# kianmcevoy/audio_analysis

Measured on AMD Instinct MI355X. Metric: IRs/sec full report (STFT+RT60bands+zplane), 48 kHz 10 s IR, higher is better.
Workload: dtype f64; 1 GPU; metrics-only full report on 256 mono synthetic IRs per GPU per step, 10 s @ 48 kHz (SURVEY.md 8d generator), H2D included: every step uploads its batch from pinned host memory (float32, 492 MB) on a copy stream under the previous step's kernels; 4 distinct batches rotate; batch_per_gpu=256, parallelism=file-sharded dp1, gather=final

## Files before the change

### audio_analysis_amd/csrc/ira_fftlong.hip

```cpp
#include <cmath>
#include <cstdlib>
#include <type_traits>

#include "ira_bandmask.h"
#include "ira_fft_lds.h"

namespace {

using ira::cplx;
typedef cplx<double> cd;

constexpr int FL_THREADS = 256;
constexpr int FL_LR = 4;

struct Geom {
  long long m;
  int n1, rad, log2q, log2n2;
  const cd* t1;
  const cd* t2;
  const cd* tf;
  int ablate;
};

__device__ __forceinline__ unsigned col_slot(const Geom& g, unsigned r) {
// ... 173 lines not shown
constexpr int FL_U = 8;

template <int MODE>
__device__ __forceinline__ RawL fetch_input(const Jobs& J, const Ctx& c, unsigned n) {
  RawL r{0.0, 0.0, 0.0, 0.0, 0.0f, 0.0f};
  if (MODE == IN_SIGNAL) {
    r.fa = c.p1[n < c.lim1 ? c.stu * n : 0u];
    r.fb = c.p2[n < c.lim2 ? c.stu * n : 0u];
  } else if (MODE == IN_SPECTRUM) {
    const unsigned k = n > c.Lu / 2 ? c.Lu - n : n;
    const unsigned kk = n < c.Lu ? k : 0u;
    const cd xk = c.s1[kk];
    r.a = xk.re; r.b = xk.im;
    if (c.two) {
      const cd x2 = c.s2[kk];
      r.c = x2.re; r.d = x2.im;
    }
  }
  return r;
}

template <int MODE>
__device__ __forceinline__ cd value_input(const Jobs& J, const Ctx& c, unsigned n, unsigned M, cd w, double h,
                                          double h2, const RawL& r, bool hann, bool second) {
  const unsigned L = c.Lu;
  if (MODE == IN_SIGNAL) {
    double v = (double)(n < c.lim1 ? r.fa : 0.0f), v2 = (double)(n < c.lim2 ? r.fb : 0.0f);
    if (hann) {
      v *= h; v2 *= h2;
    }
    if (!second) return {v * w.re, v * w.im};
    return {v * w.re - v2 * w.im, v * w.im + v2 * w.re};
  } else if (MODE == IN_FILTER) {
    unsigned m = M - n;
    if (m >= L) {
      m = n;
      if (m >= L) return {0.0, 0.0};
    }
    const cd wm = chirp((long long)m, chirp_scale((long long)L));
    return {wm.re, -wm.im};
  } else {
    if (n >= L) return {0.0, 0.0};
    const bool upper = n > L / 2;
    const unsigned k = upper ? L - n : n;
    const bool self = k == 0u || 2u * k == L;
    const cd xk = {r.a, self ? 0.0 : (upper ? -r.b : r.b)};
    const double m1 = (double)ira::mask_cut(c.b1, c.k1, (int)k, c.fv);
    const double m2 = (double)ira::mask_cut(c.b2, c.k2, (int)k, c.fv);
    cd wk;
    if (!c.two) {
      wk = ira::cmul(xk, cd{m1, m2});
    } else {
      const cd x2 = {r.c, self ? 0.0 : (upper ? -r.d : r.d)};
      wk = {xk.re * m1 - x2.im * m2, xk.im * m1 + x2.re * m2};
    }
    const cd cw = {wk.re, -wk.im};
    return ira::cmul(cw, w);
  }
}

template <int MODE>
__global__ __launch_bounds__(FL_THREADS) __attribute__((amdgpu_waves_per_eu(4, 4))) void cols_fwd_kernel(Geom g, Jobs J, cd* __restrict__ work, int C) {
  extern __shared__ __attribute__((aligned(16))) unsigned char smem_raw[];
  cd* lds = reinterpret_cast<cd*>(smem_raw);
  unsigned bx, by;
  ira::xcd_remap(bx, by);
  const int e = (int)by + J.e0;
  const Ctx ctx = job_ctx<MODE>(J, e);
  const long long L = ctx.L;
  const unsigned N1 = (unsigned)g.n1, N2 = 1u << g.log2n2;
  const long long M = g.m;
  const unsigned n2_0 = bx * C;
  const unsigned lc = 31u - (unsigned)__builtin_clz((unsigned)C), cm = (unsigned)C - 1u;
  const unsigned stride = (unsigned)g.rad * ((1u << g.log2q) + 1u);
  const int tid = threadIdx.x;
  cd* twl = lds + (size_t)C * stride;
  const cd twv = ira::tw_split_fetch<double>(g.t1, N1 >> 1, tid);
  {
    const unsigned c = tid & cm, n1_0 = tid >> lc;
    const unsigned dn = (FL_THREADS >> lc) * N2;
    const unsigned n0 = n1_0 * N2 + n2_0 + c;
    const unsigned total = N1 * (unsigned)C;
    const unsigned cnt_mine = total > (unsigned)tid ? (total - (unsigned)tid + FL_THREADS - 1) / FL_THREADS : 0u;
    auto load_phase = [&](auto known, const unsigned cnt) __attribute__((always_inline)) {
      constexpr int KNOWN = decltype(known)::value;
      constexpr int UI = (MODE == IN_SIGNAL) ? 2 * FL_UI : FL_UI;
      RawL raw[UI];
      if (cnt > 0) {
  #pragma unroll
        for (int u = 0; u < UI; ++u) {
          const unsigned j = (unsigned)u < cnt ? (unsigned)u : cnt - 1;
          raw[u] = fetch_input<MODE>(J, ctx, n0 + j * dn);
        }
      }
      cd w = {1.0, 0.0}, d = {1.0, 0.0}, e2 = {1.0, 0.0};
      long long lw1 = L, lw2 = L;
      if (MODE == IN_SIGNAL) {
        lw1 = ctx.lw1;
        lw2 = ctx.lw2;
      }
      const bool second = (KNOWN & 4) ? (MODE == IN_SIGNAL && ctx.o2 >= 0) : (KNOWN & 2) != 0;
      const bool hann = (KNOWN & 4) ? (MODE == IN_SIGNAL && J.use_hann) : (KNOWN & 1) != 0;
      const bool win1 = (KNOWN & 4) ? lw1 > 1 : true, win2 = (KNOWN & 4) ? lw2 > 1 : true;
      double hc = 1.0, hs = 0.0, rc = 1.0, rs = 0.0, hc2 = 1.0, hs2 = 0.0, rc2 = 1.0, rs2 = 0.0;
      if (MODE != IN_FILTER) {
        const ChirpScale cs = chirp_scale(L);
        const double n0d = (double)n0, dnd = (double)dn;
        w = unit_q(n0d * n0d, cs);
        d = unit_q(2.0 * n0d * dnd + dnd * dnd, cs);
        const double st = (double)ctx.st;
        const double inv1 = win1 ? 1.0 / (double)(lw1 - 1) : 0.0, inv2 = win2 ? 1.0 / (double)(lw2 - 1) : 0.0;
        {
          const int lane = tid & 63;
          const double a = lane == 0 ? chirp_angle(2.0 * dnd * dnd, cs) : (2.0 * st * dnd) * (lane == 1 ? inv1 : inv2);
          double s3, c3;
          sincospi(a, &s3, &c3);
          e2 = {lane_value(c3, 0), -lane_value(s3, 0)};
          if (hann && win1) { rs = lane_value(s3, 1); rc = lane_value(c3, 1); }
          if (hann && second && win2) { rs2 = lane_value(s3, 2); rc2 = lane_value(c3, 2); }
        }
        if (hann) {
          const double i1 = st * n0d, i2 = st * n0d + (st - 1.0);
          if (win1) sincospi((2.0 * i1 + 1.0 - (double)lw1) * inv1, &hs, &hc);
          if (second && win2) sincospi((2.0 * i2 + 1.0 - (double)lw2) * inv2, &hs2, &hc2);
        }
      }
      if (MODE == IN_SIGNAL) {
  #pragma unroll
        for (int u = 0; u < UI; ++u) asm volatile("" : "+v"(raw[u].fa), "+v"(raw[u].fb));
      }
      __builtin_amdgcn_sched_barrier(0);
      for (unsigned jb = 0; jb < cnt; jb += UI) {
        if (jb > 0) {
  #pragma unroll
          for (int u = 0; u < UI; ++u) {
            const unsigned j = jb + u < cnt ? jb + u : cnt - 1;
            raw[u] = fetch_input<MODE>(J, ctx, n0 + j * dn);
          }
        }
  #pragma unroll
        for (int u = 0; u < UI; ++u) {
          const unsigned j = jb + u;
          if (j < cnt) {
            const unsigned n1 = (tid + FL_THREADS * j) >> lc;
            const unsigned n = n0 + j * dn;
            const double h = win1 ? 0.5 + 0.5 * hc : 1.0;
            const double h2 = win2 ? 0.5 + 0.5 * hc2 : 1.0;
            lds[c * stride + col_slot(g, n1)] = (IRA_ABL(g.ablate & 1)) ? cd{(double)n, 1.0} : value_input<MODE>(J, ctx, n, (unsigned)M, w, h, h2, raw[u], hann, second);
            w = ira::cmul(w, d);
            d = ira::cmul(d, e2);
            if (hann) {
              const double nc = hc * rc - hs * rs;
              hs = hs * rc + hc * rs;
              hc = nc;
            }
            if (hann && second) {
              const double nc2 = hc2 * rc2 - hs2 * rs2;
              hs2 = hs2 * rc2 + hc2 * rs2;
              hc2 = nc2;
            }
          }
        }
      }
    };
    using std::integral_constant;
    const unsigned cnt_all = total / FL_THREADS;
    if (total % FL_THREADS != 0) {
      load_phase(integral_constant<int, 4>{}, cnt_mine);
    } else if (MODE != IN_SIGNAL) {
      load_phase(integral_constant<int, 4>{}, cnt_all);
    } else {
      const bool two = ctx.o2 >= 0;
      if (!J.use_hann) {
        if (two) load_phase(integral_constant<int, 2>{}, cnt_all); else load_phase(integral_constant<int, 0>{}, cnt_all);
      } else if (ctx.lw1 > 1 && (!two || ctx.lw2 > 1)) {
        if (two) load_phase(integral_constant<int, 3>{}, cnt_all); else load_phase(integral_constant<int, 1>{}, cnt_all);
      } else {
        load_phase(integral_constant<int, 4>{}, cnt_all);
      }
    }
  }
  ira::tw_split_put(twl, twv, tid);
  __syncthreads();
  if (!(IRA_ABL(g.ablate & 2))) {
    if (g.rad == 3) radix3_stage<false>(g, lds, twl, C, stride, tid);
    ira::lds_fft_dif<double, FL_LR, true>(lds, g.log2q, twl, (unsigned)g.rad, tid, FL_THREADS, C * g.rad, (1u << g.log2q) + 1u);
  }
  cd* w = work + (long long)e * M;
  const unsigned total_o = N1 * (unsigned)C;
  for (unsigned base = 0; base < total_o; base += FL_THREADS * FL_UI) {
    cd th[FL_UI], tl[FL_UI];
#pragma unroll
    for (int u = 0; u < FL_UI; ++u) {
      unsigned i = base + tid + FL_THREADS * u;
      i = i < total_o ? i : total_o - 1;
      const unsigned p = (n2_0 + (i & cm)) * row_k1(g, i >> lc);
      th[u] = g.t1[p >> g.log2n2];
      tl[u] = g.tf[p & (N2 - 1u)];
    }
#pragma unroll
    for (int u = 0; u < FL_UI; ++u) {
      const unsigned i = base + tid + FL_THREADS * u;
      if (i >= total_o) continue;
      const unsigned c = i & cm, r = i >> lc;
      const cd v = ira::cmul(lds[c * stride + col_slot(g, r)], ira::cmul(th[u], tl[u]));
      if ((IRA_ABL(g.ablate & 4)) && v.re != 12345.678) continue;
      w[(long long)r * N2 + n2_0 + c] = v;
    }
  }
}

template <int MODE>
__global__ __launch_bounds__(FL_THREADS) __attribute__((amdgpu_waves_per_eu(4, 4))) void rows_kernel(Geom g, Jobs J, cd* __restrict__ work, int R) {
  extern __shared__ __attribute__((aligned(16))) unsigned char smem_raw[];
  cd* lds = reinterpret_cast<cd*>(smem_raw);
  unsigned bx, by;
  ira::xcd_remap(bx, by);
  const int e = (int)by + J.e0;
  const unsigned N2 = 1u << g.log2n2;
  const long long M = g.m;
// ... 45 lines not shown
        unsigned i = base + tid + FL_THREADS * u;
        i = i < total ? i : total - 1;
        const unsigned p = (i & (N2 - 1)) * row_k1(g, r0 + (i >> g.log2n2));
        th[u] = g.t1[p >> g.log2n2];
        tl[u] = g.tf[p & (N2 - 1u)];
      }
#pragma unroll
      for (int u = 0; u < FL_UI; ++u) {
        const unsigned i = base + tid + FL_THREADS * u;
        if (i >= total) continue;
        cd t = ira::cmul(th[u], tl[u]);
        t.im = -t.im;
        const cd v = ira::cmul(lds[i], t);
        if ((IRA_ABL(g.ablate & 128)) && v.re != 12345.678) continue;
        w[i] = v;
      }
    }
  } else {
    for (unsigned i = tid; i < total; i += FL_THREADS) w[i] = lds[i];
  }
}

template <int MODE>
__global__ __launch_bounds__(FL_THREADS) __attribute__((amdgpu_waves_per_eu(4, 4))) void cols_inv_kernel(Geom g, Jobs J, const cd* __restrict__ work, int C) {
  extern __shared__ __attribute__((aligned(16))) unsigned char smem_raw[];
  cd* lds = reinterpret_cast<cd*>(smem_raw);
  unsigned bx, by;
  ira::xcd_remap(bx, by);
  const int e = (int)by + J.e0;
  long long L, out1, out2 = -1;
  bool paired = false;
  {
    const int l = J.L[e];
    if (MODE == OUT_SPECTRUM) {
      const long long x2 = J.x2off ? (long long)J.x2off[e] : -1ll, zo = J.x2off ? (long long)J.zpair_off[e] : 0ll;
      const long long so = J.spec_out_off[e];
      paired = ira::uniform(x2) >= 0;
      out1 = paired ? ira::uniform(zo) : ira::uniform(so);
    } else {
      const long long y1 = J.y1_off[e], y2 = J.y2_off[e];
      out1 = ira::uniform(y1);
      out2 = ira::uniform(y2);
    }
    L = ira::uniform(l);
  }
  const unsigned N1 = (unsigned)g.n1, N2 = 1u << g.log2n2;
  const long long M = g.m;
  const unsigned n2_0 = bx * C;
  const unsigned lc = 31u - (unsigned)__builtin_clz((unsigned)C), cm = (unsigned)C - 1u;
  const unsigned stride = (unsigned)g.rad * ((1u << g.log2q) + 1u);
  const int tid = threadIdx.x;
  const long long n_need = (MODE == OUT_SPECTRUM && !paired) ? L / 2 + 1 : L;
  const cd* w = work + (long long)e * M;
  const unsigned total = N1 * (unsigned)C;
  cd* twl = lds + (size_t)C * stride;
  const cd twv = ira::tw_split_fetch<double>(g.t1, N1 >> 1, tid);
  for (unsigned base = 0; base < total; base += FL_THREADS * FL_U) {
    cd raw[FL_U];
#pragma unroll
    for (int u = 0; u < FL_U; ++u) {
      unsigned i = base + tid + FL_THREADS * u;
      i = i < total ? i : total - 1;
      raw[u] = (IRA_ABL(g.ablate & 256)) ? cd{(double)i, 1.0} : w[(long long)(i >> lc) * N2 + n2_0 + (i & cm)];
    }
#pragma unroll
    for (int u = 0; u < FL_U; ++u) {
      const unsigned i = base + tid + FL_THREADS * u;
      if (i < total) lds[(i & cm) * stride + col_slot(g, i >> lc)] = raw[u];
    }
  }
  ira::tw_split_put(twl, twv, tid);
  __syncthreads();
  if (!(IRA_ABL(g.ablate & 32))) {
    ira::lds_fft_dit<double, FL_LR, true>(lds, g.log2q, twl, (unsigned)g.rad, true, tid, FL_THREADS, C * g.rad, (1u << g.log2q) + 1u);
    if (g.rad == 3) radix3_stage<true>(g, lds, twl, C, stride, tid);
  }
  const double inv_m = 1.0 / (double)M;
  const long long dn = (long long)(FL_THREADS >> lc) * N2;
  const long long n0 = (long long)((unsigned)tid >> lc) * N2 + n2_0 + ((unsigned)tid & cm);
  const ChirpScale cs = chirp_scale(L);
  const double n0d = (double)n0, dnd = (double)dn;
  cd cw = unit_q(n0d * n0d, cs), cdl = unit_q(2.0 * n0d * dnd + dnd * dnd, cs);
  const cd ce2 = unit_q(2.0 * dnd * dnd, cs);
  for (unsigned i = tid; i < N1 * (unsigned)C; i += FL_THREADS) {
    const unsigned c = i & cm, n1 = i >> lc;
    const long long n = (long long)n1 * N2 + n2_0 + c;
    const cd wn = cw;
    cw = ira::cmul(cw, cdl);
    cdl = ira::cmul(cdl, ce2);
    if (n >= n_need) continue;
    cd v = lds[c * stride + col_slot(g, n1)];
    if (!(IRA_ABL(g.ablate & 64))) v = ira::cmul(v, wn);
    if (MODE == OUT_SPECTRUM) {
      v.re *= inv_m; v.im *= inv_m;
      if (paired) {
        J.zpair[out1 + n] = v;
      } else {
        if (n == 0 || (2 * n == L)) v.im = 0.0;
        J.spec_out[out1 + n] = v;
      }
    } else {
      const double sc = inv_m / (double)L;
      J.y[out1 + n] = (float)(v.re * sc);
      if (out2 >= 0) J.y[out2 + n] = (float)(-v.im * sc);
    }
  }
}

__global__ __launch_bounds__(256) void pair_split_kernel(Jobs J) {
  const int e = blockIdx.y;
  if (J.x2off[e] < 0 || (J.interleave && J.interleave[e])) return;
  const long long L = J.L[e];
  const long long k = (long long)blockIdx.x * blockDim.x + threadIdx.x;
  if (k > L / 2) return;
  const cd* z = J.zpair + J.zpair_off[e];
  const long long o1 = J.spec_out_off[e], o2 = J.spec_out_off2[e];
  ira::pair_split_bin(z, L, k, J.spec_out + o1 + k, J.spec_out + o2 + k);
}

__global__ __launch_bounds__(256) void half_split_kernel(Jobs J) {
  const int e = blockIdx.y;
  if (!J.interleave[e]) return;
  const long long L = J.L[e];
  const long long k = (long long)blockIdx.x * blockDim.x + threadIdx.x;
  if (k > L) return;
  const cd* z = J.zpair + J.zpair_off[e];
  J.spec_out[J.spec_out_off[e] + k] = ira::half_split_bin(z, L, k);
}

struct Split { int rad, log2q, log2n2; };

bool split_of(long long m, Split* out) {
  if (m < 16 || m > (1ll << 22)) return false;
  int rad = 1;
  if (m % 3 == 0) { rad = 3; m /= 3; }
  if ((m & (m - 1)) != 0) return false;
  int log2p = 0;
  while ((1ll << log2p) < m) ++log2p;
  int lq;
  if (rad == 1) {
    const int forced = ira_tune_int("IRA_FFT_SPLIT", 0);
    lq = (log2p + 1) / 2;
    if (forced > 0) lq = forced;
    if (lq < 2) lq = 2;
    if (lq > log2p - 2) lq = log2p - 2;
    if (log2p - lq > 13) lq = log2p - 13;
  } else {
    if (log2p < 5) return false;
    lq = (log2p - 1) / 2;
    { const int forced = ira_tune_int("IRA_FFT_SPLIT3", 0); if (forced >= 2 && forced <= log2p - 2) lq = forced; }
    if (log2p - lq > 13) lq = log2p - 13;
  }
  out->rad = rad; out->log2q = lq; out->log2n2 = log2p - lq;
  return true;
}

struct Plan {
  Geom g;
  int C, R;
  size_t lds_cols, lds_rows;
  int C3; size_t lds_cols3;
};

int32_t make_plan(int32_t m, const void* t1, const void* t2, const void* tf, Plan* p) {
  Split sp;
  if (!split_of(m, &sp)) return IRA_E_SIZE;
  p->g.m = m;
// ... 139 lines not shown
```

### audio_analysis_amd/csrc/ira_spectrum.hip

```cpp
#include <cmath>

#include "ira_fft_reg.h"
#include "ira_log.h"
#include "ira_reduce.h"

namespace {

typedef ira::cplx<double> cd;
constexpr double kPi = 3.14159265358979323846;

constexpr int ATAN_TAB = 64;

__device__ __attribute__((noinline)) double atan2_lib(double y, double x) { return atan2(y, x); }
__device__ __attribute__((noinline)) double fmod_lib(double a, double b) { return fmod(a, b); }
__device__ __attribute__((noinline)) double exp10_lib(double y) { return exp10(y); }
__device__ __attribute__((noinline)) cd twiddle_lib(long long k, long long l) {
  double sn, cs;
  sincospi(-(double)(k % (2 * l)) / (double)l, &sn, &cs);
  return {cs, sn};
}
__device__ __attribute__((noinline)) float db_lib(double re, double im, double floor_lin) {
  const double a = hypot(re, im);
  const double m = (a != a) ? a : fmax(a, floor_lin);
  return (float)(20.0 * log10(m));
}

__device__ __forceinline__ void build_atan_table(double* tab, int tid) {
  if (tid <= ATAN_TAB) tab[tid] = atan((double)tid * (1.0 / ATAN_TAB));
}

__device__ __forceinline__ double atan2_table(double y, double x, const double* tab) {
  const double ax = fabs(x), ay = fabs(y);
  const double mx = fmax(ax, ay), mn = fmin(ax, ay);
  if (!(ax > 1.0e-300 && ay > 1.0e-300 && ax < 1.0e300 && ay < 1.0e300)) return atan2_lib(y, x);
  const double t = mn / mx;
  const int k = (int)(t * (double)ATAN_TAB + 0.5);
  const double t0 = (double)k * (1.0 / ATAN_TAB);
  const double r = (t - t0) / fma(t, t0, 1.0);
  const double r2 = r * r;
  double s = fma(r2, 1.0 / 9.0, -1.0 / 7.0);
  s = fma(r2, s, 0.2);
  s = fma(r2, s, -1.0 / 3.0);
  s = fma(r2, s, 1.0);
  double a = fma(r, s, tab[k]);
  if (ay > ax) a = 1.5707963267948966 - a;
  if (x < 0.0) a = kPi - a;
  return copysign(a, y);
}

__device__ __forceinline__ double unwrap_correction(double prev, double cur) {
  const double dd = cur - prev;
  const double period = 2.0 * kPi;
  double a = dd + kPi;
  double md;
  if (a >= 0.0 && a < period) md = a;
  else if (a >= period && a < 2.0 * period) md = a - period;
  else if (a < 0.0 && a > -period) md = a;
  else md = fmod_lib(a, period);
  if (md != 0.0) {
    if (md < 0.0) md += period;
  } else {
    md = 0.0;
  }
  double ddmod = md + (-kPi);
  if (ddmod == -kPi && dd > 0.0) ddmod = kPi;
  double corr = ddmod - dd;
  if (fabs(dd) < kPi) corr = 0.0;
  return corr;
}

__device__ __forceinline__ cd packed_bin(cd zk, cd zl, double cs, double sn, bool edge) {
  const auto [ev, od] = ira::hermitian_parts(zk, zl);
  cd v = {ev.re + (cs * od.re - sn * od.im), ev.im + (cs * od.im + sn * od.re)};
  if (edge) v.im = 0.0;
  return v;
}

__device__ __forceinline__ float bin_db(cd v, double floor_lin, double floor_p, float floor_db32,
                                        const ira::LogTabEntry* ltab) {
  const double p = v.re * v.re + v.im * v.im;
  if (p > 1.0e-280 && p < 1.0e280 && floor_lin > 1.0e-140) {
    return p > floor_p ? (float)(3.0102999566398120 * ira::log2_table(p, ltab)) : floor_db32;
  }
  return db_lib(v.re, v.im, floor_lin);
}

__global__ __launch_bounds__(256) void mag_phase_kernel(const cd* __restrict__ spec, const int64_t* __restrict__ spec_off,
                                 const int32_t* __restrict__ L, double floor_lin, float* __restrict__ mag_db,
                                 const int64_t* __restrict__ mag_off, double* __restrict__ phase,
                                 const int64_t* __restrict__ phase_off, const int32_t* __restrict__ packed) {
  __shared__ ira::LogTabEntry ltab[ira::LOGTAB_N];
  __shared__ double atab[ATAN_TAB + 1];
  ira::build_log_table(ltab, threadIdx.x);
  build_atan_table(atab, threadIdx.x);
  __syncthreads();
  const int e = blockIdx.y;
  const long long nb = (long long)L[e] / 2 + 1;
  const cd* s = spec + spec_off[e];
  float* mo = mag_db + mag_off[e];
  double* po = phase ? phase + phase_off[e] : nullptr;
  const double floor_p = floor_lin * floor_lin;
  const float floor_db32 = (float)(20.0 * log10(floor_lin));
  const bool pk = packed != nullptr && ira::uniform(packed[e]) != 0;
  const long long l = (long long)L[e] / 2;
  const long long k_first = (long long)blockIdx.x * blockDim.x + threadIdx.x, k_step = (long long)gridDim.x * blockDim.x;
  double cs = 1.0, sn = 0.0, rc = 1.0, rs = 0.0;
  if (pk) {
    sincospi(-(double)(k_first < nb ? k_first : 0) / (double)l, &sn, &cs);
    sincospi(-(double)(k_step % (2 * l)) / (double)l, &rs, &rc);
  }
  for (long long k = k_first; k < nb; k += k_step) {
    cd v;
    if (pk) {
      v = packed_bin(s[k == l ? 0 : k], s[(k == 0 || k == l) ? 0 : l - k], cs, sn, k == 0 || k == l);
      const double nc = cs * rc - sn * rs;
      sn = sn * rc + cs * rs;
      cs = nc;
    } else {
      v = s[k];
    }
    mo[k] = bin_db(v, floor_lin, floor_p, floor_db32, ltab);
// ... 226 lines not shown
      __syncthreads();
    }
    if (compacted) {
#pragma unroll
      for (int r = 0; r < OS_MAX_RANKS; ++r) {
        if (!lead[r]) continue;
        const int li = list_of[r];
        const int cnt = list_n[li] < OS_CAP ? list_n[li] : OS_CAP;
        for (int i = tid; i < cnt; i += OS_THREADS) {
          const unsigned long long k = os_key(list[li][i]);
          if ((k & himask) == pf[r]) atomicAdd(&hist[r][(unsigned int)(k >> shift) & 255u], 1u);
        }
      }
    } else {
      for (long long it = 0; it < trips; ++it) {
        unsigned long long kk[OS_U];
        bool vv[OS_U];
#pragma unroll
        for (int u = 0; u < OS_U; ++u) {
          const long long i = (it * OS_U + u) * OS_THREADS + tid;
          vv[u] = i < n;
          kk[u] = os_key(v[vv[u] ? i : n - 1]);
        }
#pragma unroll
        for (int u = 0; u < OS_U; ++u) {
          const bool valid = vv[u];
          const unsigned long long k = kk[u];
          const unsigned int digit = (unsigned int)(k >> shift) & 255u;
#pragma unroll
          for (int r = 0; r < OS_MAX_RANKS; ++r) {
            if (!lead[r]) continue;
            const bool m = valid && (k & himask) == pf[r];
            const unsigned long long act = __ballot(m);
            if (act == 0ull) continue;
            const int first = __ffsll((long long)act) - 1;
            const unsigned int d0 = (unsigned int)__shfl((int)digit, first, 64);
            const unsigned long long same = __ballot(m && digit == d0);
            if (lane == first) atomicAdd(&hist[r][d0], (unsigned int)__popcll(same));
            if (m && digit != d0) atomicAdd(&hist[r][digit], 1u);
          }
        }
      }
    }
    __syncthreads();
    for (int r = 0; r < nranks; ++r) {
      const int l = leader[r];
      const long long rem = remaining[r];
      const long long c = tid < 256 ? (long long)hist[l][tid] : 0ll;
      long long in_wave;
      long long incl = ira::wave_prefix(c, lane, in_wave);
      if (tid < 256 && lane == 63) scan_tot[tid >> 6] = incl;
      __syncthreads();
      if (tid < 256) {
        for (int w = 0; w < (tid >> 6); ++w) incl += scan_tot[w];
        const long long excl = incl - c;
        if ((excl <= rem && rem < incl) || (tid == 255 && rem >= incl)) {
          remaining[r] = rem - excl;
          bucket[r] = c;
          prefix[r] = prefix[r] | ((unsigned long long)tid << shift);
        }
      }
      __syncthreads();
    }
  }
  if (tid < nranks) o[tid] = os_unkey(prefix[tid]);
}

constexpr int ST_THREADS = 1024;

struct StatsAcc {
  double cnt = 0.0, sfl = 0.0, sl = 0.0;
  unsigned long long best = 0ull;
  unsigned long long near = ~0ull;
  long long first_in;
  float near_db = 0.0f;
};
struct StatsScratch {
  double red[3][ST_THREADS / IRA_WAVE];
  unsigned long long kred[2][ST_THREADS / IRA_WAVE];
  long long lred[ST_THREADS / IRA_WAVE];
  float dred[ST_THREADS / IRA_WAVE];
};

__device__ __forceinline__ void stats_bin(StatsAcc& a, long long k, float db, double val, float f_min, float f_max,
                                          float probe_hz, const double* etab) {
  const float f = (float)((double)k * val);
  const float d = fabsf(f - probe_hz);
  const unsigned long long nk = ((unsigned long long)__float_as_uint(d) << 32) | (unsigned long long)(uint32_t)k;
  a.near_db = nk < a.near ? db : a.near_db;
  a.near = nk < a.near ? nk : a.near;
  if (f >= f_min && f <= f_max) {
    uint32_t uu = ira::float_key(db);
    if (db != db) uu = 0xFFFFFFFFu;
    const unsigned long long key = ((unsigned long long)uu << 32) | (unsigned long long)(0xFFFFFFFFu - (uint32_t)k);
    a.best = key > a.best ? key : a.best;
    const double y = (double)db * 0.05;
    const double lin = fabs(y) < 15.0 ? ira::exp10_table(y, etab) : exp10_lib(y);
    a.cnt += 1.0; a.sfl += (double)f * lin; a.sl += lin;
    a.first_in = k < a.first_in ? k : a.first_in;
  }
}

__device__ __forceinline__ void stats_finish(StatsAcc a, StatsScratch& sc, long long n, double val, double* o) {
  const int t = threadIdx.x, lane = t & 63, wave = t >> 6;
  a.cnt = ira::wave_sum(a.cnt); a.sfl = ira::wave_sum(a.sfl); a.sl = ira::wave_sum(a.sl);
#pragma unroll
  for (int o2 = 32; o2 > 0; o2 >>= 1) {
    const unsigned long long ob = __shfl_xor(a.best, o2, 64);
    a.best = ob > a.best ? ob : a.best;
    const unsigned long long on = __shfl_xor(a.near, o2, 64);
    const float od = __shfl_xor(a.near_db, o2, 64);
    a.near_db = on < a.near ? od : a.near_db;
    a.near = on < a.near ? on : a.near;
    const long long of = __shfl_xor(a.first_in, o2, 64);
    a.first_in = of < a.first_in ? of : a.first_in;
  }
  if (lane == 0) {
    sc.red[0][wave] = a.cnt; sc.red[1][wave] = a.sfl; sc.red[2][wave] = a.sl;
    sc.kred[0][wave] = a.best; sc.kred[1][wave] = a.near; sc.lred[wave] = a.first_in; sc.dred[wave] = a.near_db;
  }
  __syncthreads();
  if (t == 0) {
    a.cnt = a.sfl = a.sl = 0.0;
    for (int w = 0; w < ST_THREADS / IRA_WAVE; ++w) {
      a.cnt += sc.red[0][w]; a.sfl += sc.red[1][w]; a.sl += sc.red[2][w];
      a.best = sc.kred[0][w] > a.best ? sc.kred[0][w] : a.best;
      a.near_db = sc.kred[1][w] < a.near ? sc.dred[w] : a.near_db;
      a.near = sc.kred[1][w] < a.near ? sc.kred[1][w] : a.near;
      a.first_in = sc.lred[w] < a.first_in ? sc.lred[w] : a.first_in;
    }
    const long long pk = (a.cnt > 0.0) ? (long long)(0xFFFFFFFFu - (uint32_t)(a.best & 0xFFFFFFFFull)) : 0;
    o[0] = a.cnt;
    o[1] = (double)pk;
    o[2] = (double)(float)((double)pk * val);
    o[3] = a.sfl; o[4] = a.sl;
    o[5] = a.first_in < n ? (double)(float)((double)a.first_in * val) : 0.0;
    o[6] = (double)(long long)(a.near & 0xFFFFFFFFull);
    o[7] = (double)a.near_db;
  }
}

__global__ __launch_bounds__(ST_THREADS) void stats_kernel(const float* __restrict__ mag_db,
                                                           const int64_t* __restrict__ mag_off,
                                                           const int32_t* __restrict__ L,
                                                           const double* __restrict__ freq_val, float f_min, float f_max,
                                                           float probe_hz, double* __restrict__ out) {
  __shared__ StatsScratch sc;
  __shared__ double etab[ira::EXPTAB_N];
  const int e = blockIdx.x;
  const long long n = (long long)L[e] / 2 + 1;
  const float* m = mag_db + mag_off[e];
  const double val = freq_val[e];
  const int t = threadIdx.x;
  ira::build_exp_table(etab, t);
  __syncthreads();
  StatsAcc acc;
  acc.first_in = n;
  constexpr int ST_U = 16;
  for (long long k0 = t; k0 < n; k0 += (long long)ST_THREADS * ST_U) {
    float dbv[ST_U];
#pragma unroll
    for (int u = 0; u < ST_U; ++u) {
      const long long k = k0 + (long long)ST_THREADS * u;
      dbv[u] = m[k < n ? k : n - 1];
    }
#pragma unroll
    for (int u = 0; u < ST_U; ++u) {
      const long long k = k0 + (long long)ST_THREADS * u;
      if (k >= n) continue;
      stats_bin(acc, k, dbv[u], val, f_min, f_max, probe_hz, etab);
    }
  }
  stats_finish(acc, sc, n, val, out + (int64_t)e * 8);
}

constexpr int SF_TWQ = 512;
constexpr int SF_STAGE = 2;

template <bool DB, bool PHASE>
__global__ __launch_bounds__(UW_THREADS) void spectrum_finish_kernel(
    const cd* __restrict__ spec, const int64_t* __restrict__ spec_off, const int32_t* __restrict__ L, double floor_lin,
    const int32_t* __restrict__ packed, float* __restrict__ mag_db, const int64_t* __restrict__ out_off, int do_unwrap,
    double out_scale, float* __restrict__ phase32, double* __restrict__ phase64, double* __restrict__ wrapped64,
    const double* __restrict__ freq_val, float f_min, float f_max, float probe_hz, double* __restrict__ stats) {
  static_assert(ST_THREADS == UW_THREADS, "the statistics' thread mapping is the tile's load mapping");
  __shared__ ira::LogTabEntry ltab[ira::LOGTAB_N];
  __shared__ double atab[ATAN_TAB + 1];
  __shared__ double etab[ira::EXPTAB_N];
  __shared__ StatsScratch sc;
  __shared__ cd twq[SF_TWQ];
  __shared__ double ph_tile[UW_TILE];
  __shared__ double wave_tot[UW_THREADS / IRA_WAVE];
  __shared__ double tile_total, prev_last;
  const int e = blockIdx.x;
  const int t = threadIdx.x, lane = t & 63, wave = t >> 6;
  const long long len = ira::uniform(L[e]);
  const long long n = len / 2 + 1, l = len / 2;
  const cd* s = spec + ira::uniform(spec_off[e]);
  const long long oo = ira::uniform(out_off[e]);
  const bool pk = packed != nullptr && ira::uniform(packed[e]) != 0 && l > 0;
  const bool want_stats = DB && stats != nullptr;
  const double val = want_stats ? ira::uniform(freq_val[e]) : 0.0;
  const double floor_p = floor_lin * floor_lin;
  const float floor_db32 = (float)(20.0 * log10(floor_lin));
  if constexpr (DB) ira::build_log_table(ltab, t);
  if constexpr (PHASE) build_atan_table(atab, t);
  if (want_stats) ira::build_exp_table(etab, t);
  double wt_c = 1.0, wt_s = 0.0;
  auto build_twq = [&](long long q0) {
    const long long k = (q0 + t) * UW_THREADS;
    if (t < SF_TWQ && k < n) twq[t] = twiddle_lib(k, l);
  };
  if (pk) {
    const cd wt = twiddle_lib(t, l);
    wt_c = wt.re;
    wt_s = wt.im;
    build_twq(0);
  }
  if (t == 0) { tile_total = 0.0; prev_last = 0.0; }
  __syncthreads();
  StatsAcc acc;
  acc.first_in = n;
  cd nza[SF_STAGE], nzb[SF_STAGE];
  auto load_stage = [&](long long first) {
#pragma unroll
    for (int r = 0; r < SF_STAGE; ++r) {
      const long long k = first + t + (long long)UW_THREADS * r;
      nza[r] = {0.0, 0.0};
      nzb[r] = {0.0, 0.0};
      if (k < n) {
        if (pk) {
          nza[r] = s[k == l ? 0 : k];
          nzb[r] = s[(k == 0 || k == l) ? 0 : l - k];
        } else {
          nza[r] = s[k];
        }
      }
    }
  };
  load_stage(0);
  for (long long base = 0; base < n; base += UW_TILE) {
    if (pk && base > 0 && base % ((long long)SF_TWQ * UW_THREADS) == 0) {
      __syncthreads();
      build_twq(base / UW_THREADS);
      __syncthreads();
    }
    const long long qb = base / ((long long)SF_TWQ * UW_THREADS) * SF_TWQ;
#pragma unroll 1
    for (int h = 0; h < UW_PER / SF_STAGE; ++h) {
      const long long first = base + (long long)h * SF_STAGE * UW_THREADS;
      cd za[SF_STAGE], zb[SF_STAGE];
#pragma unroll
      for (int r = 0; r < SF_STAGE; ++r) { za[r] = nza[r]; zb[r] = nzb[r]; }
      if (first + SF_STAGE * UW_THREADS < n) load_stage(first + SF_STAGE * UW_THREADS);
#pragma unroll
      for (int r = 0; r < SF_STAGE; ++r) {
        const int j = t + UW_THREADS * (h * SF_STAGE + r);
        const long long k = base + j;
        double ph = 0.0;
        if (k < n) {
          cd v = za[r];
          if (pk) {
            const cd w = twq[k / UW_THREADS - qb];
            const double cs = w.re * wt_c - w.im * wt_s;
            const double sn = w.im * wt_c + w.re * wt_s;
            v = packed_bin(za[r], zb[r], cs, sn, k == 0 || k == l);
          }
          if constexpr (DB) {
            const float db = bin_db(v, floor_lin, floor_p, floor_db32, ltab);
            mag_db[oo + k] = db;
            if (want_stats) stats_bin(acc, k, db, val, f_min, f_max, probe_hz, etab);
          }
          if constexpr (PHASE) {
            ph = atan2_table(v.im, v.re, atab);
            if (wrapped64) wrapped64[oo + k] = ph;
          }
        }
        if constexpr (PHASE) ph_tile[j] = ph;
      }
    }
    if constexpr (PHASE) {
      __syncthreads();
      const double carry = tile_total;
      const long long i0 = base + (long long)UW_PER * t;
      double c[UW_PER], v[UW_PER];
      double prev = t == 0 ? prev_last : ph_tile[UW_PER * t - 1];
#pragma unroll
      for (int r = 0; r < UW_PER; ++r) v[r] = ph_tile[UW_PER * t + r];
#pragma unroll
      for (int r = 0; r < UW_PER; ++r) {
        const long long i = i0 + r;
        c[r] = (do_unwrap && i >= 1 && i < n) ? unwrap_correction(prev, v[r]) : 0.0;
        prev = v[r];
      }
      const double add = unwrap_scan(c, carry, wave_tot, lane, wave);
#pragma unroll
      for (int r = 0; r < UW_PER; ++r) {
        const long long i = i0 + r;
        if (i < n) {
          const double u = v[r] + (c[r] + add);
          if (phase32) phase32[oo + i] = (float)(u * out_scale);
          if (phase64) phase64[oo + i] = u;
        }
      }
      if (t == UW_THREADS - 1) { tile_total = c[3] + add; prev_last = v[3]; }
    }
  }
  if (want_stats) stats_finish(acc, sc, n, val, stats + (int64_t)e * 8);
}

constexpr int LS_MAX = 2048;
constexpr int LS_THREADS = 256;

__device__ __forceinline__ double ls_freq(long long k, double fstep) { return (double)(float)((double)k * fstep); }

__global__ __launch_bounds__(LS_THREADS) void log_smooth_kernel(float* __restrict__ mag, const int64_t* __restrict__ off,
                                                                const int32_t* __restrict__ stride_a,
                                                                const int32_t* __restrict__ k_lo_a,
                                                                const int32_t* __restrict__ nsel_a,
                                                                const double* __restrict__ fstep_a,
                                                                const double* __restrict__ lg_lo, const double* __restrict__ lg_hi,
                                                                const int32_t* __restrict__ count_a, int window,
                                                                int through_f32) {
  __shared__ double xg[LS_MAX], on[LS_MAX], sm[LS_MAX];
  const int c = blockIdx.x, tid = threadIdx.x;
  const int count = count_a[c], nsel = nsel_a[c], k_lo = k_lo_a[c];
  const long long stride = stride_a[c];
  const double fstep = fstep_a[c], a = lg_lo[c], b = lg_hi[c];
  if (count < 2 || count > LS_MAX || nsel < 1) return;
  float* m = mag + off[c];
  const double step = (b - a) / (double)(count - 1);
  for (int g = tid; g < count; g += LS_THREADS) {
    const double y = (g == count - 1) ? b : (double)g * step + a;
    const double x = exp2(y);
    xg[g] = x;
    double v;
    const double f0 = ls_freq(k_lo, fstep), fl = ls_freq((long long)k_lo + nsel - 1, fstep);
    if (nsel == 1 || x <= f0) v = (double)m[(long long)k_lo * stride];
    else if (x >= fl) v = (double)m[(long long)(k_lo + nsel - 1) * stride];
    else {
      int lo = 0, hi = nsel - 1;
      while (hi - lo > 1) {
        const int mid = (lo + hi) >> 1;
        if (ls_freq((long long)k_lo + mid, fstep) <= x) lo = mid; else hi = mid;
      }
      const double x0 = ls_freq((long long)k_lo + lo, fstep), x1 = ls_freq((long long)k_lo + lo + 1, fstep);
      const double y0 = (double)m[(long long)(k_lo + lo) * stride], y1 = (double)m[(long long)(k_lo + lo + 1) * stride];
      const double slope = (y1 - y0) / (x1 - x0);
      v = slope * (x - x0) + y0;
    }
    on[g] = through_f32 ? (double)(float)v : v;
  }
  __syncthreads();
  const double inv_w = 1.0 / (double)window;
  const int h = (window - 1) / 2;
  for (int g = tid; g < count; g += LS_THREADS) {
    int j0 = g + h - (window - 1), j1 = g + h;
    if (j0 < 0) j0 = 0;
    if (j1 > count - 1) j1 = count - 1;
    double acc = 0.0;
    for (int j = j0; j <= j1; ++j) acc += on[j] * inv_w;
    sm[g] = through_f32 ? (double)(float)acc : acc;
  }
  __syncthreads();
  for (int i = tid; i < nsel; i += LS_THREADS) {
    const double x = ls_freq((long long)k_lo + i, fstep);
    double v;
    if (x <= xg[0]) v = sm[0];
    else if (x >= xg[count - 1]) v = sm[count - 1];
    else {
      int lo = 0, hi = count - 1;
      while (hi - lo > 1) {
        const int mid = (lo + hi) >> 1;
        if (xg[mid] <= x) lo = mid; else hi = mid;
      }
      const double slope = (sm[lo + 1] - sm[lo]) / (xg[lo + 1] - xg[lo]);
      v = slope * (x - xg[lo]) + sm[lo];
    }
    m[(long long)(k_lo + i) * stride] = (float)v;
  }
}

}

extern "C" int32_t ira_spectrum_mag_phase(const double* spec_dev, const int64_t* spec_off_dev, const int32_t* L_dev,
// ... 110 lines not shown
```

Before: 17730 IRs/s.

## Skip zero-padding loads and unneeded output rows; cheapen atan2 and index math

In the long FFT input stage, threads now stop fetching the signal past the data region and write zeros directly to LDS for padded rows. In the output stage, loop trip counts are clamped to the rows actually needed. Separately, the table-based atan2 uses a hardware reciprocal and a division-reduced formulation, and the spectrum kernel switches its index math from 64-bit to 32-bit with precomputed output base pointers. The approximate reciprocal may slightly change phase rounding, and the int indices assume bin counts fit in 32 bits.

```diff
diff --git a/audio_analysis_amd/csrc/ira_fftlong.hip b/audio_analysis_amd/csrc/ira_fftlong.hip
--- a/audio_analysis_amd/csrc/ira_fftlong.hip
+++ b/audio_analysis_amd/csrc/ira_fftlong.hip
@@ -279,16 +279,35 @@
     const unsigned n0 = n1_0 * N2 + n2_0 + c;
     const unsigned total = N1 * (unsigned)C;
     const unsigned cnt_mine = total > (unsigned)tid ? (total - (unsigned)tid + FL_THREADS - 1) / FL_THREADS : 0u;
-    auto load_phase = [&](auto known, const unsigned cnt) __attribute__((always_inline)) {
+    unsigned pad_j = ~0u;
+    static_assert(FL_THREADS == 256, "the shift by 8 - lc below divides by FL_THREADS / C");
+    if (MODE == IN_SIGNAL && !(IRA_ABL(g.ablate & 1))) {
+      const unsigned data = ctx.lim1 > ctx.lim2 ? ctx.lim1 : ctx.lim2;
+      const unsigned rows_data = data > n2_0 ? (data - n2_0 + N2 - 1u) >> g.log2n2 : 0u;
+      const unsigned row_min = ira::uniform(n1_0);
+      pad_j = rows_data > row_min ? (rows_data - row_min + (FL_THREADS >> lc) - 1u) >> (8u - lc) : 0u;
+    }
+    auto load_phase = [&](auto known, const unsigned cnt_own) __attribute__((always_inline)) {
       constexpr int KNOWN = decltype(known)::value;
+      const unsigned cnt = cnt_own < pad_j ? cnt_own : pad_j;
       constexpr int UI = (MODE == IN_SIGNAL) ? 2 * FL_UI : FL_UI;
       RawL raw[UI];
-      if (cnt > 0) {
+      const unsigned cnt_w = MODE == IN_SIGNAL ? ira::uniform(cnt) : 0u;
+      if (MODE == IN_SIGNAL) {
+  #pragma unroll
+        for (int u = 0; u < UI; ++u) {
+          raw[u] = RawL{0.0, 0.0, 0.0, 0.0, 0.0f, 0.0f};
+          if ((unsigned)u < cnt_w) raw[u] = fetch_input<MODE>(J, ctx, n0 + ((unsigned)u < cnt ? (unsigned)u : (cnt ? cnt - 1 : 0u)) * dn);
+        }
+      } else if (cnt > 0) {
   #pragma unroll
         for (int u = 0; u < UI; ++u) {
           const unsigned j = (unsigned)u < cnt ? (unsigned)u : cnt - 1;
           raw[u] = fetch_input<MODE>(J, ctx, n0 + j * dn);
         }
+      }
+      if (MODE == IN_SIGNAL) {
+        for (unsigned j = cnt; j < cnt_own; ++j) lds[c * stride + col_slot(g, (tid + FL_THREADS * j) >> lc)] = cd{0.0, 0.0};
       }
       cd w = {1.0, 0.0}, d = {1.0, 0.0}, e2 = {1.0, 0.0};
       long long lw1 = L, lw2 = L;
@@ -332,7 +351,7 @@
   #pragma unroll
           for (int u = 0; u < UI; ++u) {
             const unsigned j = jb + u < cnt ? jb + u : cnt - 1;
-            raw[u] = fetch_input<MODE>(J, ctx, n0 + j * dn);
+            if (MODE != IN_SIGNAL || jb + u < cnt_w) raw[u] = fetch_input<MODE>(J, ctx, n0 + j * dn);
           }
         }
   #pragma unroll
@@ -544,7 +563,15 @@
   const double n0d = (double)n0, dnd = (double)dn;
   cd cw = unit_q(n0d * n0d, cs), cdl = unit_q(2.0 * n0d * dnd + dnd * dnd, cs);
   const cd ce2 = unit_q(2.0 * dnd * dnd, cs);
-  for (unsigned i = tid; i < N1 * (unsigned)C; i += FL_THREADS) {
+  const unsigned need_u = (unsigned)n_need;
+  const unsigned rows_need = need_u > n2_0 ? (need_u - n2_0 + N2 - 1u) >> g.log2n2 : 0u;
+  const unsigned row_min = ira::uniform((unsigned)tid >> lc);
+  static_assert(FL_THREADS == 256, "the shift by 8 - lc divides by FL_THREADS / C");
+  const unsigned j_need = rows_need > row_min ? (rows_need - row_min + (FL_THREADS >> lc) - 1u) >> (8u - lc) : 0u;
+  const unsigned j_all = (total + FL_THREADS - 1u) / FL_THREADS;
+  const unsigned j_end = j_need < j_all ? j_need : j_all;
+  const bool whole = total % FL_THREADS == 0;
+  for (unsigned j = 0, i = tid; j < j_end && (whole || i < total); ++j, i += FL_THREADS) {
     const unsigned c = i & cm, n1 = i >> lc;
     const long long n = (long long)n1 * N2 + n2_0 + c;
     const cd wn = cw;
diff --git a/audio_analysis_amd/csrc/ira_spectrum.hip b/audio_analysis_amd/csrc/ira_spectrum.hip
--- a/audio_analysis_amd/csrc/ira_spectrum.hip
+++ b/audio_analysis_amd/csrc/ira_spectrum.hip
@@ -33,10 +33,9 @@
   const double ax = fabs(x), ay = fabs(y);
   const double mx = fmax(ax, ay), mn = fmin(ax, ay);
   if (!(ax > 1.0e-300 && ay > 1.0e-300 && ax < 1.0e300 && ay < 1.0e300)) return atan2_lib(y, x);
-  const double t = mn / mx;
-  const int k = (int)(t * (double)ATAN_TAB + 0.5);
+  const int k = (int)((mn * __builtin_amdgcn_rcp(mx)) * (double)ATAN_TAB + 0.5);
   const double t0 = (double)k * (1.0 / ATAN_TAB);
-  const double r = (t - t0) / fma(t, t0, 1.0);
+  const double r = fma(-t0, mx, mn) / fma(t0, mn, mx);
   const double r2 = r * r;
   double s = fma(r2, 1.0 / 9.0, -1.0 / 7.0);
   s = fma(r2, s, 0.2);
@@ -429,7 +428,8 @@
   float dred[ST_THREADS / IRA_WAVE];
 };
 
-__device__ __forceinline__ void stats_bin(StatsAcc& a, long long k, float db, double val, float f_min, float f_max,
+template <typename K>
+__device__ __forceinline__ void stats_bin(StatsAcc& a, K k, float db, double val, float f_min, float f_max,
                                           float probe_hz, const double* etab) {
   const float f = (float)((double)k * val);
   const float d = fabsf(f - probe_hz);
@@ -545,6 +545,11 @@
   const long long n = len / 2 + 1, l = len / 2;
   const cd* s = spec + ira::uniform(spec_off[e]);
   const long long oo = ira::uniform(out_off[e]);
+  const int nb = (int)n, lh = (int)l;
+  float* const mo = DB ? mag_db + oo : nullptr;
+  double* const wo = wrapped64 ? wrapped64 + oo : nullptr;
+  float* const p32 = phase32 ? phase32 + oo : nullptr;
+  double* const p64 = phase64 ? phase64 + oo : nullptr;
   const bool pk = packed != nullptr && ira::uniform(packed[e]) != 0 && l > 0;
   const bool want_stats = DB && stats != nullptr;
   const double val = want_stats ? ira::uniform(freq_val[e]) : 0.0;
@@ -569,16 +574,16 @@
   StatsAcc acc;
   acc.first_in = n;
   cd nza[SF_STAGE], nzb[SF_STAGE];
-  auto load_stage = [&](long long first) {
+  auto load_stage = [&](int first) {
 #pragma unroll
     for (int r = 0; r < SF_STAGE; ++r) {
-      const long long k = first + t + (long long)UW_THREADS * r;
+      const int k = first + t + UW_THREADS * r;
       nza[r] = {0.0, 0.0};
       nzb[r] = {0.0, 0.0};
-      if (k < n) {
+      if (k < nb) {
         if (pk) {
-          nza[r] = s[k == l ? 0 : k];
-          nzb[r] = s[(k == 0 || k == l) ? 0 : l - k];
+          nza[r] = s[k == lh ? 0 : k];
+          nzb[r] = s[(k == 0 || k == lh) ? 0 : lh - k];
         } else {
           nza[r] = s[k];
         }
@@ -586,41 +591,41 @@
     }
   };
   load_stage(0);
-  for (long long base = 0; base < n; base += UW_TILE) {
-    if (pk && base > 0 && base % ((long long)SF_TWQ * UW_THREADS) == 0) {
+  for (int base = 0; base < nb; base += UW_TILE) {
+    if (pk && base > 0 && base % (SF_TWQ * UW_THREADS) == 0) {
       __syncthreads();
       build_twq(base / UW_THREADS);
       __syncthreads();
     }
-    const long long qb = base / ((long long)SF_TWQ * UW_THREADS) * SF_TWQ;
+    const int qb = base / (SF_TWQ * UW_THREADS) * SF_TWQ;
 #pragma unroll 1
     for (int h = 0; h < UW_PER / SF_STAGE; ++h) {
-      const long long first = base + (long long)h * SF_STAGE * UW_THREADS;
+      const int first = base + h * SF_STAGE * UW_THREADS;
       cd za[SF_STAGE], zb[SF_STAGE];
 #pragma unroll
       for (int r = 0; r < SF_STAGE; ++r) { za[r] = nza[r]; zb[r] = nzb[r]; }
-      if (first + SF_STAGE * UW_THREADS < n) load_stage(first + SF_STAGE * UW_THREADS);
+      if (first + SF_STAGE * UW_THREADS < nb) load_stage(first + SF_STAGE * UW_THREADS);
 #pragma unroll
       for (int r = 0; r < SF_STAGE; ++r) {
         const int j = t + UW_THREADS * (h * SF_STAGE + r);
-        const long long k = base + j;
+        const int k = base + j;
         double ph = 0.0;
-        if (k < n) {
+        if (k < nb) {
           cd v = za[r];
           if (pk) {
-            const cd w = twq[k / UW_THREADS - qb];
+            const cd w = twq[base / UW_THREADS + (h * SF_STAGE + r) - qb];
             const double cs = w.re * wt_c - w.im * wt_s;
             const double sn = w.im * wt_c + w.re * wt_s;
-            v = packed_bin(za[r], zb[r], cs, sn, k == 0 || k == l);
+            v = packed_bin(za[r], zb[r], cs, sn, k == 0 || k == lh);
           }
           if constexpr (DB) {
             const float db = bin_db(v, floor_lin, floor_p, floor_db32, ltab);
-            mag_db[oo + k] = db;
+            mo[k] = db;
             if (want_stats) stats_bin(acc, k, db, val, f_min, f_max, probe_hz, etab);
           }
           if constexpr (PHASE) {
             ph = atan2_table(v.im, v.re, atab);
-            if (wrapped64) wrapped64[oo + k] = ph;
+            if (wo) wo[k] = ph;
           }
         }
         if constexpr (PHASE) ph_tile[j] = ph;
@@ -629,25 +634,25 @@
     if constexpr (PHASE) {
       __syncthreads();
       const double carry = tile_total;
-      const long long i0 = base + (long long)UW_PER * t;
+      const int i0 = base + UW_PER * t;
       double c[UW_PER], v[UW_PER];
       double prev = t == 0 ? prev_last : ph_tile[UW_PER * t - 1];
 #pragma unroll
       for (int r = 0; r < UW_PER; ++r) v[r] = ph_tile[UW_PER * t + r];
 #pragma unroll
       for (int r = 0; r < UW_PER; ++r) {
-        const long long i = i0 + r;
-        c[r] = (do_unwrap && i >= 1 && i < n) ? unwrap_correction(prev, v[r]) : 0.0;
+        const int i = i0 + r;
+        c[r] = (do_unwrap && i >= 1 && i < nb) ? unwrap_correction(prev, v[r]) : 0.0;
         prev = v[r];
       }
       const double add = unwrap_scan(c, carry, wave_tot, lane, wave);
 #pragma unroll
       for (int r = 0; r < UW_PER; ++r) {
-        const long long i = i0 + r;
-        if (i < n) {
+        const int i = i0 + r;
+        if (i < nb) {
           const double u = v[r] + (c[r] + add);
-          if (phase32) phase32[oo + i] = (float)(u * out_scale);
-          if (phase64) phase64[oo + i] = u;
+          if (p32) p32[i] = (float)(u * out_scale);
+          if (p64) p64[i] = u;
         }
       }
       if (t == UW_THREADS - 1) { tile_total = c[3] + add; prev_last = v[3]; }
```

Measured after the change: 17630 IRs/s. About the same (-0.6%).
